# ghostop14/gr-clenabled

Hardware: AMD Instinct MI355X
Metric: MSamples/sec (complex-float) through clFFT 4096 fwd + window + shift (higher is better)
Workload: dtype f32; 1 GPU; BASELINE configs[1]: forward clFFT 4096-pt complex, blackman window + fftshift, 16384 frames/step/GPU device-resident (1 GiB in+out); fft_size=4096, parallelism=replica-per-gpu x1

## Files before the change

### gr-clenabled_amd/csrc/fft_mr.h

```cpp
#pragma once
#include <vector>

#include "common.h"

struct MrPass {
    int radix, ns, nb;
    unsigned m_nb, m_ns;
    int tw_off;
};

struct MrPlan {
    int n = 0, npass = 0;
    int threads = 0;
    int frames = 0;
    int lds_bytes = 0;
    int variant = 0;
    int per_thread = 0;
    MrPass pass[12];
    void *d_tw = nullptr;
};

bool mi355_fft_mr_plan(int n, int sign, int variant, MrPlan *plan, std::vector<float> *tw);

int mi355_fft_mr_tune(MrPlan *plan, mi355_ctx *ctx, int sign, const float *window_dev, float *best_ms);
int mi355_fft_mr_cached_variant(int n);
void mi355_fft_mr_remember(const MrPlan &plan);

int mi355_fft_mr_launch(const MrPlan &plan, mi355_ctx *ctx, int sign, const void *in, void *out, const float *window, int nframes, int shift,
                        int real_in, hipStream_t st);

bool mi355_fft_mr_pfb_ok(const MrPlan &plan, int sign, int K, int M, int nsteps);
int mi355_fft_mr_pfb_launch(const MrPlan &plan, mi355_ctx *ctx, const void *in, void *out, const float *taps, int K, int M, int nsteps, hipStream_t st);
struct MrSynthGeo {
    int threads = 0, frames = 0;
    int nreg = 0, rs = 0;
    int taps_lds = 0, lds_bytes = 0;
};
bool mi355_fft_mr_synth_ok(const MrPlan &plan, int sign, int M, int T, MrSynthGeo *g);
int mi355_fft_mr_synth_launch(const MrPlan &plan, const MrSynthGeo &g, mi355_ctx *ctx, const void *in, void *out, const float *taps_pad,
                              const int *ch_map, int nmap, int T, long long nframes, hipStream_t st);
struct mi355_fft;
const MrPlan *mi355_fft_mr_plan_of(const mi355_fft *h, int *sign);

struct MrTilePlan {
    int n = 0, n1 = 0, n2 = 0;
    MrPlan a, b;
    void *d_twn = nullptr;
};
bool mi355_fft_mr_tile_plan(int n, int sign, MrTilePlan *tp, std::vector<float> *twa, std::vector<float> *twb);
int mi355_fft_mr_tile_launch(const MrTilePlan &tp, mi355_ctx *ctx, int sign, const void *in, void *ws, void *out, const float *window, int nframes,
                             int shift, int real_in, hipStream_t st);
```

### gr-clenabled_amd/csrc/fft_mr.hip

```cpp
#include "fft_mr.h"

#include <cmath>
#include <cstdlib>
#include <map>
#include <mutex>
#include <utility>

#include "fft_core.hpp"
#include "synth_fir.hpp"

using namespace fftc;

namespace {

typedef float f2v __attribute__((ext_vector_type(2)));
constexpr int kVals = 16;
constexpr int kMaxPass = 12;

struct MrArgs {
    const void *in;
    c32 *out;
    const float *window;
    const c32 *tw;
    int n, nframes, frames, npass, in_rot, out_rot, real_in;
    int copy_in = 0;
    int copy_out = 0;
    unsigned m_n = 0;
    int tw_lds = 0, ntw = 0;
    int dbg = 0;
    int fs_shift = 0;
    long long range_len = 0;
    long long ngroups;
    MrPass pass[kMaxPass];
};

__device__ __forceinline__ int slot(int i) { return i + (i >> 5); }

template <int R> __host__ __device__ constexpr int fac_a() { return R == 6 ? 2 : R == 9 ? 3 : R == 10 ? 2 : R == 12 ? 4 : R == 14 ? 2 : R == 15 ? 3 : 1; }
template <int R> __host__ __device__ constexpr int out_index(int s)
{
    if (R == 8 || R == 16) return orev<R>(s);
    if (fac_a<R>() > 1) return s / (R / fac_a<R>()) + fac_a<R>() * (s % (R / fac_a<R>()));
    return s;
}

template <int R> struct Roots;
template <> struct Roots<6> {
    static constexpr float c[6] = {1.000000000e+00f, 5.000000000e-01f, -5.000000000e-01f, -1.000000000e+00f, -5.000000000e-01f, 5.000000000e-01f};
    static constexpr float s[6] = {0.000000000e+00f, 8.660254038e-01f, 8.660254038e-01f, 1.224646799e-16f, -8.660254038e-01f, -8.660254038e-01f};
};
template <> struct Roots<9> {
    static constexpr float c[9] = {1.000000000e+00f, 7.660444431e-01f, 1.736481777e-01f, -5.000000000e-01f, -9.396926208e-01f, -9.396926208e-01f, -5.000000000e-01f, 1.736481777e-01f, 7.660444431e-01f};
    static constexpr float s[9] = {0.000000000e+00f, 6.427876097e-01f, 9.848077530e-01f, 8.660254038e-01f, 3.420201433e-01f, -3.420201433e-01f, -8.660254038e-01f, -9.848077530e-01f, -6.427876097e-01f};
};
template <> struct Roots<10> {
    static constexpr float c[10] = {1.000000000e+00f, 8.090169944e-01f, 3.090169944e-01f, -3.090169944e-01f, -8.090169944e-01f, -1.000000000e+00f, -8.090169944e-01f, -3.090169944e-01f, 3.090169944e-01f, 8.090169944e-01f};
    static constexpr float s[10] = {0.000000000e+00f, 5.877852523e-01f, 9.510565163e-01f, 9.510565163e-01f, 5.877852523e-01f, 1.224646799e-16f, -5.877852523e-01f, -9.510565163e-01f, -9.510565163e-01f, -5.877852523e-01f};
};
template <> struct Roots<12> {
    static constexpr float c[12] = {1.000000000e+00f, 8.660254038e-01f, 5.000000000e-01f, 6.123233996e-17f, -5.000000000e-01f, -8.660254038e-01f, -1.000000000e+00f, -8.660254038e-01f, -5.000000000e-01f, -1.836970199e-16f, 5.000000000e-01f, 8.660254038e-01f};
    static constexpr float s[12] = {0.000000000e+00f, 5.000000000e-01f, 8.660254038e-01f, 1.000000000e+00f, 8.660254038e-01f, 5.000000000e-01f, 1.224646799e-16f, -5.000000000e-01f, -8.660254038e-01f, -1.000000000e+00f, -8.660254038e-01f, -5.000000000e-01f};
};
template <> struct Roots<14> {
    static constexpr float c[14] = {1.000000000e+00f, 9.009688679e-01f, 6.234898019e-01f, 2.225209340e-01f, -2.225209340e-01f, -6.234898019e-01f, -9.009688679e-01f, -1.000000000e+00f, -9.009688679e-01f, -6.234898019e-01f, -2.225209340e-01f, 2.225209340e-01f, 6.234898019e-01f, 9.009688679e-01f};
    static constexpr float s[14] = {0.000000000e+00f, 4.338837391e-01f, 7.818314825e-01f, 9.749279122e-01f, 9.749279122e-01f, 7.818314825e-01f, 4.338837391e-01f, 1.224646799e-16f, -4.338837391e-01f, -7.818314825e-01f, -9.749279122e-01f, -9.749279122e-01f, -7.818314825e-01f, -4.338837391e-01f};
};
template <> struct Roots<15> {
    static constexpr float c[15] = {1.000000000e+00f, 9.135454576e-01f, 6.691306064e-01f, 3.090169944e-01f, -1.045284633e-01f, -5.000000000e-01f, -8.090169944e-01f, -9.781476007e-01f, -9.781476007e-01f, -8.090169944e-01f, -5.000000000e-01f, -1.045284633e-01f, 3.090169944e-01f, 6.691306064e-01f, 9.135454576e-01f};
    static constexpr float s[15] = {0.000000000e+00f, 4.067366431e-01f, 7.431448255e-01f, 9.510565163e-01f, 9.945218954e-01f, 8.660254038e-01f, 5.877852523e-01f, 2.079116908e-01f, -2.079116908e-01f, -5.877852523e-01f, -8.660254038e-01f, -9.945218954e-01f, -9.510565163e-01f, -7.431448255e-01f, -4.067366431e-01f};
};

template <> struct Roots<11> {
    static constexpr float c[11] = {1.000000000e+00f, 8.412535328e-01f, 4.154150130e-01f, -1.423148383e-01f, -6.548607339e-01f, -9.594929736e-01f, -9.594929736e-01f, -6.548607339e-01f, -1.423148383e-01f, 4.154150130e-01f, 8.412535328e-01f};
    static constexpr float s[11] = {0.000000000e+00f, 5.406408175e-01f, 9.096319954e-01f, 9.898214419e-01f, 7.557495744e-01f, 2.817325568e-01f, -2.817325568e-01f, -7.557495744e-01f, -9.898214419e-01f, -9.096319954e-01f, -5.406408175e-01f};
};
template <> struct Roots<13> {
    static constexpr float c[13] = {1.000000000e+00f, 8.854560257e-01f, 5.680647467e-01f, 1.205366803e-01f, -3.546048870e-01f, -7.485107482e-01f, -9.709418174e-01f, -9.709418174e-01f, -7.485107482e-01f, -3.546048870e-01f, 1.205366803e-01f, 5.680647467e-01f, 8.854560257e-01f};
    static constexpr float s[13] = {0.000000000e+00f, 4.647231720e-01f, 8.229838659e-01f, 9.927088741e-01f, 9.350162427e-01f, 6.631226582e-01f, 2.393156643e-01f, -2.393156643e-01f, -6.631226582e-01f, -9.350162427e-01f, -9.927088741e-01f, -8.229838659e-01f, -4.647231720e-01f};
};

template <int R, int SIGN> __device__ __forceinline__ void dft(c32 *v)
{
    if constexpr (R == 2) bfly2<SIGN>(v[0], v[1]);
    else if constexpr (R == 4) bfly4<SIGN>(v[0], v[1], v[2], v[3]);
    else if constexpr (R == 8) bfly8<SIGN>(v);
    else if constexpr (R == 16) bfly16<SIGN>(v);
    else if constexpr (R == 3) {
        constexpr float s3 = 0.86602540378443864676f;
        const c32 t = v[1] + v[2], d = rot90<SIGN>(scale(v[1] - v[2], s3));
        const c32 m = mk(v[0].x - 0.5f * t.x, v[0].y - 0.5f * t.y);
        v[0] = v[0] + t;
        v[1] = m + d;
        v[2] = m - d;
    } else if constexpr (R == 5) {
        constexpr float c1 = 0.30901699437494742410f, c2 = -0.80901699437494742410f, s1 = 0.95105651629515357212f, s2 = 0.58778525229247312917f;
        const c32 t1 = v[1] + v[4], t2 = v[2] + v[3], t3 = v[1] - v[4], t4 = v[2] - v[3];
        const c32 a1 = mk(v[0].x + c1 * t1.x + c2 * t2.x, v[0].y + c1 * t1.y + c2 * t2.y);
        const c32 a2 = mk(v[0].x + c2 * t1.x + c1 * t2.x, v[0].y + c2 * t1.y + c1 * t2.y);
        const c32 b1 = rot90<SIGN>(mk(s1 * t3.x + s2 * t4.x, s1 * t3.y + s2 * t4.y));
        const c32 b2 = rot90<SIGN>(mk(s2 * t3.x - s1 * t4.x, s2 * t3.y - s1 * t4.y));
        v[0] = v[0] + t1 + t2;
        v[1] = a1 + b1;
        v[4] = a1 - b1;
        v[2] = a2 + b2;
        v[3] = a2 - b2;
    } else if constexpr (fac_a<R>() > 1) {
        constexpr int A = fac_a<R>(), B = R / A;
#pragma unroll
        for (int b = 0; b < B; b++) {
            c32 t[A];
#pragma unroll
            for (int q = 0; q < A; q++) t[q] = v[B * q + b];
            dft<A, SIGN>(t);
#pragma unroll
            for (int k1 = 0; k1 < A; k1++) {
                c32 y = t[k1];
                if (b * k1 != 0) {
                    constexpr float sg = SIGN < 0 ? -1.f : 1.f;
                    y = cmul(y, mk(Roots<R>::c[(b * k1) % R], sg * Roots<R>::s[(b * k1) % R]));
                }
                v[B * k1 + b] = y;
            }
        }
#pragma unroll
        for (int k1 = 0; k1 < A; k1++) dft<B, SIGN>(&v[B * k1]);
    } else if constexpr (R == 11 || R == 13) {
        constexpr int H = (R - 1) / 2;
        c32 t[H], u[H];
#pragma unroll
        for (int j = 0; j < H; j++) {
            t[j] = v[j + 1] + v[R - 1 - j];
            u[j] = v[j + 1] - v[R - 1 - j];
        }
        c32 x0 = v[0], sum = v[0];
#pragma unroll
        for (int j = 0; j < H; j++) sum = sum + t[j];
        v[0] = sum;
#pragma unroll
        for (int k = 1; k <= H; k++) {
            c32 ak = x0, bk = mk(0.f, 0.f);
#pragma unroll
            for (int j = 1; j <= H; j++) {
                const float c = Roots<R>::c[(j * k) % R], sn = Roots<R>::s[(j * k) % R];
                ak = mk(ak.x + c * t[j - 1].x, ak.y + c * t[j - 1].y);
                bk = mk(bk.x + sn * u[j - 1].x, bk.y + sn * u[j - 1].y);
            }
            const c32 jb = rot90<SIGN>(bk);
            v[k] = ak + jb;
            v[R - k] = ak - jb;
        }
    } else {
        static_assert(R == 7, "radix");
        constexpr float c1 = 0.62348980185873353053f, c2 = -0.22252093395631440429f, c3 = -0.90096886790241912624f;
        constexpr float s1 = 0.78183148246802980871f, s2 = 0.97492791218182360702f, s3 = 0.43388373911755812048f;
        const c32 t1 = v[1] + v[6], t2 = v[2] + v[5], t3 = v[3] + v[4], u1 = v[1] - v[6], u2 = v[2] - v[5], u3 = v[3] - v[4];
        const c32 a1 = mk(v[0].x + c1 * t1.x + c2 * t2.x + c3 * t3.x, v[0].y + c1 * t1.y + c2 * t2.y + c3 * t3.y);
        const c32 a2 = mk(v[0].x + c2 * t1.x + c3 * t2.x + c1 * t3.x, v[0].y + c2 * t1.y + c3 * t2.y + c1 * t3.y);
        const c32 a3 = mk(v[0].x + c3 * t1.x + c1 * t2.x + c2 * t3.x, v[0].y + c3 * t1.y + c1 * t2.y + c2 * t3.y);
        const c32 b1 = rot90<SIGN>(mk(s1 * u1.x + s2 * u2.x + s3 * u3.x, s1 * u1.y + s2 * u2.y + s3 * u3.y));
        const c32 b2 = rot90<SIGN>(mk(s2 * u1.x - s3 * u2.x - s1 * u3.x, s2 * u1.y - s3 * u2.y - s1 * u3.y));
        const c32 b3 = rot90<SIGN>(mk(s3 * u1.x - s1 * u2.x + s2 * u3.x, s3 * u1.y - s1 * u2.y + s2 * u3.y));
        v[0] = v[0] + t1 + t2 + t3;
        v[1] = a1 + b1;
        v[6] = a1 - b1;
        v[2] = a2 + b2;
        v[5] = a2 - b2;
        v[3] = a3 + b3;
        v[4] = a3 - b3;
    }
}

template <int R, int SIGN, int MODE, bool TWL = false>
__device__ __forceinline__ void mr_pass(const MrArgs &a, const MrPass &ps, c32 *lds, int tid, long long group)
{
    const int TH = blockDim.x;
    constexpr int B = kVals / R;
    c32 v[B][R], w1[B];
    const int n = a.n, nb = ps.nb, nbt = a.frames * nb;
#pragma unroll
    for (int i = 0; i < B; i++) {
        const int b = tid + TH * i;
        const int fr = (int)__umulhi((unsigned)b, ps.m_nb), bb = b - fr * nb;
        if constexpr (MODE == 1 || MODE == 2) {
            const int k = bb - (int)__umulhi((unsigned)bb, ps.m_ns) * ps.ns;
            if constexpr (TWL) w1[i] = b < nbt ? lds[a.tw_lds + ps.tw_off + k] : mk(1.f, 0.f);
            else
            w1[i] = b < nbt ? a.tw[ps.tw_off + k] : mk(1.f, 0.f);
        }
        if (b < nbt) {
            if constexpr (MODE == 0) {
                const long long frame = group * a.frames + fr;
                const bool live = frame < a.nframes;
#pragma unroll
                for (int r = 0; r < R; r++) {
                    int src = bb + r * nb + a.in_rot;
                    if (src >= n) src -= n;
                    c32 x = mk(0.f, 0.f);
                    if (live) {
                        if (a.real_in) x = mk(((const float *)a.in)[(size_t)frame * n + src], 0.f);
                        else {
                            const f2v t = __builtin_nontemporal_load((const f2v *)a.in + (size_t)frame * n + src);
                            x = mk(t.x, t.y);
                        }
                        const float w = a.window[src];
                        x = mk(x.x * w, x.y * w);
                    }
                    v[i][r] = x;
                }
            } else {
                const int base = fr * n + bb;
#pragma unroll
                for (int r = 0; r < R; r++) v[i][r] = lds[slot(base + r * nb)];
            }
        }
    }
    if constexpr (MODE != 0) __syncthreads();
#pragma unroll
    for (int i = 0; i < B; i++) {
        const int b = tid + TH * i;
        if (b < nbt) {
            const int fr = (int)__umulhi((unsigned)b, ps.m_nb), bb = b - fr * nb;
            int g = bb, k = 0;
            if constexpr (MODE == 1 || MODE == 2) {
                g = (int)__umulhi((unsigned)bb, ps.m_ns);
                k = bb - g * ps.ns;
                c32 sq[4];
                sq[0] = w1[i];
#pragma unroll
                for (int q = 1; q < 4; q++) sq[q] = (R > (1 << q)) ? cmul(sq[q - 1], sq[q - 1]) : sq[q - 1];
#pragma unroll
                for (int r = 1; r < R; r++) {
                    c32 t = mk(1.f, 0.f);
                    bool first = true;
#pragma unroll
                    for (int q = 0; q < 4; q++)
                        if ((r >> q) & 1) {
                            t = first ? sq[q] : cmul(t, sq[q]);
                            first = false;
                        }
                    v[i][r] = cmul(v[i][r], t);
                }
            }
            dft<R, SIGN>(v[i]);
            if constexpr (MODE == 2) {
                const long long frame = a.fs_shift ? group + (fr >> a.fs_shift) * a.range_len + (fr & ((1 << a.fs_shift) - 1)) : group * a.frames + fr;
                if (frame < a.nframes) {
#pragma unroll
                    for (int s = 0; s < R; s++) {
                        int p = k + out_index<R>(s) * ps.ns - a.out_rot;
                        if (p < 0) p += n;
                        f2v z;
                        z.x = v[i][s].x;
                        z.y = v[i][s].y;
                        __builtin_nontemporal_store(z, (f2v *)a.out + (size_t)frame * n + p);
                    }
                }
            } else {
                const int base = fr * n + g * ps.ns * R + k;
#pragma unroll
                for (int s = 0; s < R; s++) lds[slot(base + out_index<R>(s) * ps.ns)] = v[i][s];
            }
        }
    }
    if constexpr (MODE != 2) __syncthreads();
}

template <int SIGN>
__global__ __launch_bounds__(1024) void k_fft_mr(const MrArgs a)
{
    extern __shared__ __attribute__((aligned(16))) c32 mr_lds[];
    const int tid0 = threadIdx.x;
#define MR_PASS(MODE, P)                                                                        \
    switch (a.pass[P].radix) {                                                                  \
    case 2: mr_pass<2, SIGN, MODE>(a, a.pass[P], mr_lds, tid, group); break;                \
    case 3: mr_pass<3, SIGN, MODE>(a, a.pass[P], mr_lds, tid, group); break;                \
    case 4: mr_pass<4, SIGN, MODE>(a, a.pass[P], mr_lds, tid, group); break;                \
    case 5: mr_pass<5, SIGN, MODE>(a, a.pass[P], mr_lds, tid, group); break;                \
    case 7: mr_pass<7, SIGN, MODE>(a, a.pass[P], mr_lds, tid, group); break;                \
    case 6: mr_pass<6, SIGN, MODE>(a, a.pass[P], mr_lds, tid, group); break;                    \
    case 9: mr_pass<9, SIGN, MODE>(a, a.pass[P], mr_lds, tid, group); break;                    \
    case 10: mr_pass<10, SIGN, MODE>(a, a.pass[P], mr_lds, tid, group); break;                  \
    case 11: mr_pass<11, SIGN, MODE>(a, a.pass[P], mr_lds, tid, group); break;                  \
    case 13: mr_pass<13, SIGN, MODE>(a, a.pass[P], mr_lds, tid, group); break;                  \
    case 12: mr_pass<12, SIGN, MODE>(a, a.pass[P], mr_lds, tid, group); break;                  \
    case 14: mr_pass<14, SIGN, MODE>(a, a.pass[P], mr_lds, tid, group); break;                  \
    case 15: mr_pass<15, SIGN, MODE>(a, a.pass[P], mr_lds, tid, group); break;                  \
    case 8: mr_pass<8, SIGN, MODE>(a, a.pass[P], mr_lds, tid, group); break;                \
    default: mr_pass<16, SIGN, MODE>(a, a.pass[P], mr_lds, tid, group); break;              \
    }
    for (long long group = blockIdx.x; group < a.ngroups; group += gridDim.x) {
        int tid = tid0;
        asm volatile("" : "+v"(tid));
        if (a.copy_in) {
            const int tot = a.frames * a.n;
            for (int idx = tid0; idx < tot; idx += blockDim.x) {
                const int fr = (int)__umulhi((unsigned)idx, a.m_n), q = idx - fr * a.n;
                int i = q - a.in_rot;
                if (i < 0) i += a.n;
                c32 x = mk(0.f, 0.f);
                if (group * a.frames + fr < a.nframes) {
                    const size_t at = (size_t)group * a.frames * a.n + idx;
                    if (a.real_in) x = mk(((const float *)a.in)[at], 0.f);
                    else {
                        const f2v t = __builtin_nontemporal_load((const f2v *)a.in + at);
                        x = mk(t.x, t.y);
                    }
                    const float w = a.window[q];
                    x = mk(x.x * w, x.y * w);
                }
                mr_lds[slot(fr * a.n + i)] = x;
            }
            __syncthreads();
            MR_PASS(3, 0)
        } else {
            MR_PASS(0, 0)
        }
        for (int p = 1; p < a.npass - 1; p++) { MR_PASS(1, p) }
        if (a.copy_out) {
            MR_PASS(1, a.npass - 1)
            const int tot = a.frames * a.n;
            for (int idx = tid0; idx < tot; idx += blockDim.x) {
                const int fr = (int)__umulhi((unsigned)idx, a.m_n);
                int p = idx - fr * a.n + a.out_rot;
                if (p >= a.n) p -= a.n;
                if (group * a.frames + fr < a.nframes) {
                    const c32 v = mr_lds[slot(fr * a.n + p)];
                    f2v z;
                    z.x = v.x;
                    z.y = v.y;
                    __builtin_nontemporal_store(z, (f2v *)a.out + (size_t)group * a.frames * a.n + idx);
                }
            }
            __syncthreads();
        } else {
            MR_PASS(2, a.npass - 1)
        }
    }
#undef MR_PASS
}


struct PfbMr {
    const c32 *in;
    const float *taps;
    int K, M, Q, nsteps, direct;
    unsigned m_M, m_run;
};

template <int SIGN, int PMAX, int FS>
__global__ __launch_bounds__(512) void k_pfb_mr(const MrArgs a, const PfbMr f)
{
    extern __shared__ __attribute__((aligned(16))) c32 mr_lds[];
    const int tid0 = threadIdx.x;
    const int q = (int)__umulhi((unsigned)tid0, f.m_M), j = tid0 - q * f.M;
    const bool arm = q < f.Q;
// ... 380 lines not shown
}
}

namespace {
bool plan_len(int n, int sign, int variant, bool column_of_a_tile, MrPlan *plan, std::vector<float> *tw);
}

bool mi355_fft_mr_plan(int n, int sign, int variant, MrPlan *plan, std::vector<float> *tw)
{
    if ((n & (n - 1)) == 0) return false;
    return plan_len(n, sign, variant, false, plan, tw);
}

namespace {
bool plan_len(int n, int sign, int variant, bool column_of_a_tile, MrPlan *plan, std::vector<float> *tw)
{
    if (n < 4 || n > 16 * 1024) return false;
    Factorisation fz;
    {
        int cur[kMaxPass];
        search(n, n, 0, 0, kVals, variant ? 14 : 0, cur, &fz);
    }
    if (fz.np > kMaxPass) return false;
    int radix[kMaxPass], np = 0;
    for (int pass = 0; pass < 2; pass++)
        for (int i = 0; i < fz.np; i++) {
            const bool pow2 = (fz.r[i] & (fz.r[i] - 1)) == 0;
            if ((pass == 0) != pow2) radix[np++] = fz.r[i];
        }
    int per_thread = kVals;
    for (int p = 0; p < np; p++) {
        const int v = (kVals / radix[p]) * radix[p];
        if (v < per_thread) per_thread = v;
    }
    int th = 0, frames = 0;
    long long best = 0;
    for (int w : {8, 6, 5, 4, 3, 2, 1}) {
        int t = w == 1 ? 1024 : 1536 / w / 64 * 64;
        long long f = (long long)t * per_thread / n;
        const long long lds_vals = (160 * 1024 / w / 8 - 1) * 32 / 33;
        if (f > lds_vals / n) f = lds_vals / n;
        if (f < 1) continue;
        if (w * f * n > best) {
            best = w * f * n;
            th = t;
            frames = (int)f;
        }
    }
    if (column_of_a_tile) {
        th = (int)((16LL * n + per_thread - 1) / per_thread + 63) / 64 * 64;
        frames = 16;
        if (th > 1024) return false;
    } else
    if (const char *e = getenv("MI355_FFT_MR_THREADS")) {
        const int t = atoi(e), f = getenv("MI355_FFT_MR_FRAMES") ? atoi(getenv("MI355_FFT_MR_FRAMES")) : 1;
        if (t >= 64 && t <= 1024 && t % 64 == 0 && f >= 1 && (long long)f * n <= (long long)t * per_thread) { th = t; frames = f; }
    }
    if (!th) return false;
    plan->n = n;
    plan->npass = np;
    plan->threads = th;
    plan->frames = frames;
    plan->lds_bytes = (plan->frames * n + (plan->frames * n >> 5) + 1) * 8;
    plan->per_thread = per_thread;
    plan->variant = variant;
    tw->clear();
    int ns = 1;
    for (int p = 0; p < np; p++) {
        MrPass &ps = plan->pass[p];
        ps.radix = radix[p];
        ps.ns = ns;
        ps.nb = n / radix[p];
        ps.m_nb = magic(ps.nb);
        ps.m_ns = ns > 1 ? magic(ns) : 0;
        ps.tw_off = (int)(tw->size() / 2);
        if (p > 0)
            for (int k = 0; k < ns; k++) {
                const double a = sign * 2.0 * M_PI * (double)k / ((double)ns * radix[p]);
                tw->push_back((float)cos(a));
                tw->push_back((float)sin(a));
            }
        ns *= radix[p];
    }
    return true;
}
}

namespace {
int lds_bytes_for(int n, int frames) { return (frames * n + (frames * n >> 5) + 1) * 8; }

int launch_with(const MrPlan &plan, int threads, int frames, mi355_ctx *ctx, int sign, const void *in, void *out, const float *window, int nframes,
                int shift, int real_in, hipStream_t st)
{
    MrArgs a;
    a.in = in;
    a.out = (c32 *)out;
    a.window = window;
    a.tw = (const c32 *)plan.d_tw;
    a.n = plan.n;
    a.nframes = nframes;
    a.frames = frames;
    a.npass = plan.npass;
    a.in_rot = (sign > 0 && shift) ? plan.n / 2 : 0;
    a.out_rot = (sign < 0 && shift) ? (plan.n + 1) / 2 : 0;
    a.real_in = real_in;
    a.ngroups = ((long long)nframes + frames - 1) / frames;
    for (int p = 0; p < plan.npass; p++) a.pass[p] = plan.pass[p];
    static const bool no_copy_out = getenv("MI355_FFT_MR_NO_COPY_OUT") != nullptr;
    static const int copy_ns = getenv("MI355_FFT_MR_COPY_OUT_NS") ? atoi(getenv("MI355_FFT_MR_COPY_OUT_NS")) : 32;
    if (no_copy_out) MI355_SWITCH_NOTE(ctx, "MI355_FFT_MR_NO_COPY_OUT", "k_fft_mr with the passes' own loads and stores");
    if (copy_ns != 32) MI355_SWITCH_NOTE(ctx, "MI355_FFT_MR_COPY_OUT_NS", "another run length below which k_fft_mr stores through LDS");
    a.copy_out = plan.pass[plan.npass - 1].ns < copy_ns && !no_copy_out;
    a.m_n = magic(plan.n);
    static const int copy_nb = getenv("MI355_FFT_MR_COPY_IN_NB") ? atoi(getenv("MI355_FFT_MR_COPY_IN_NB")) : 16;
    if (copy_nb != 16) MI355_SWITCH_NOTE(ctx, "MI355_FFT_MR_COPY_IN_NB", "another run length below which k_fft_mr loads through LDS");
    a.copy_in = plan.pass[0].nb < copy_nb && !no_copy_out;
    const int cus = mi355_cus(ctx);
    const int lds_bytes = lds_bytes_for(plan.n, frames);
    int per_cu = (160 * 1024) / lds_bytes;
    if (per_cu > 2048 / threads) per_cu = 2048 / threads;
    if (per_cu < 1) per_cu = 1;
    long long grid = (long long)cus * per_cu;
    if (grid > a.ngroups) grid = a.ngroups;
    static std::map<int, bool> lds_ok;
    static std::mutex lds_ok_lock;
    {
        std::lock_guard<std::mutex> g(lds_ok_lock);
        const int which = ctx->device * 2 + (sign < 0 ? 0 : 1);
        if (!lds_ok[which]) {
            if (sign < 0) MI355_HIP(hipFuncSetAttribute((const void *)k_fft_mr<-1>, hipFuncAttributeMaxDynamicSharedMemorySize, 160 * 1024));
            else MI355_HIP(hipFuncSetAttribute((const void *)k_fft_mr<1>, hipFuncAttributeMaxDynamicSharedMemorySize, 160 * 1024));
            lds_ok[which] = true;
        }
    }
#define MR_LAUNCH(SG) hipLaunchKernelGGL((k_fft_mr<SG>), dim3((unsigned)grid), dim3(threads), lds_bytes, st, a)
    if (sign < 0) MR_LAUNCH(-1); else MR_LAUNCH(1);
#undef MR_LAUNCH
    MI355_HIP(hipGetLastError());
    return MI355_OK;
}

std::mutex g_tuned_lock;
struct Tuned { int variant, threads, frames; };
std::map<int, Tuned> g_tuned;
}

int mi355_fft_mr_launch(const MrPlan &plan, mi355_ctx *ctx, int sign, const void *in, void *out, const float *window, int nframes, int shift,
                        int real_in, hipStream_t st)
{
    if (nframes <= 0) return MI355_OK;
    return launch_with(plan, plan.threads, plan.frames, ctx, sign, in, out, window, nframes, shift, real_in, st);
}

bool mi355_fft_mr_pfb_ok(const MrPlan &plan, int sign, int K, int M, int nsteps)
{
    if (!plan.n || plan.n != M || sign <= 0 || plan.npass < 2 || getenv("MI355_PFB_NO_MR_FUSED")) return false;
    const int P = (K + M - 1) / M;
    return P <= 32 && M <= 512 && (long long)plan.per_thread * 512 >= 8LL * M && nsteps >= 1;
}

int mi355_fft_mr_pfb_launch(const MrPlan &plan, mi355_ctx *ctx, const void *in, void *out, const float *taps, int K, int M, int nsteps, hipStream_t st)
{
    constexpr int FS = 8, FS_SHIFT = 3;
    const int P = (K + M - 1) / M;
    static const int th_env = getenv("MI355_PFB_MR_THREADS") ? atoi(getenv("MI355_PFB_MR_THREADS")) : 0;
    auto ranges_of = [&](int th) { const long long byv = (long long)th * plan.per_thread / (FS * M); const int byt = th / M; return (int)(byv < byt ? byv : byt); };
    if (th_env) MI355_SWITCH_NOTE(ctx, "MI355_PFB_MR_THREADS", "k_pfb_mr with a forced workgroup size");
    int th = 512;
    if (th_env >= 64 && th_env <= 512 && th_env % 64 == 0 && ranges_of(th_env) >= 1) th = th_env;
    const int Q = ranges_of(th);
    if (Q < 1) return MI355_ERR_INVALID_ARG;
    const int cus = mi355_cus(ctx);
    int ntw = 0;
    for (int p = 1; p < plan.npass; p++) ntw += plan.pass[p].ns;
    const int tw_lds = lds_bytes_for(M, Q * FS) / 8;
    const int pmax = P <= 8 ? 8 : P <= 16 ? 16 : 32;
    const int lds_bytes = (tw_lds + ntw) * 8 + pmax * M * 4;
    static const int wg_env = getenv("MI355_PFB_MR_WG_PER_CU") ? atoi(getenv("MI355_PFB_MR_WG_PER_CU")) : 0;
    if (wg_env > 0) MI355_SWITCH_NOTE(ctx, "MI355_PFB_MR_WG_PER_CU", "k_pfb_mr with a forced number of workgroups per CU");
    int per_cu = wg_env > 0 ? wg_env : (pmax == 8 ? 16 : 12) / (th / 64);
    if (per_cu > (160 * 1024) / lds_bytes) per_cu = (160 * 1024) / lds_bytes;
    if (per_cu < 1) per_cu = 1;
    long long len = (nsteps + (long long)cus * Q - 1) / ((long long)cus * Q);
    if (len >= 8LL * P) {
        const long long nr = (long long)cus * per_cu * Q;
        len = (nsteps + nr - 1) / nr;
        if (len < 8LL * P) len = 8LL * P;
    }
    len = (len + FS - 1) / FS * FS;
    const long long grid = (nsteps + len * Q - 1) / (len * Q);
    MrArgs a;
    a.in = nullptr;
    a.out = (c32 *)out;
    a.window = nullptr;
    a.tw = (const c32 *)plan.d_tw;
    a.n = M;
    a.nframes = nsteps;
    a.frames = Q * FS;
    a.npass = plan.npass;
    a.in_rot = a.out_rot = a.real_in = 0;
    a.fs_shift = FS_SHIFT;
    a.range_len = len;
    a.tw_lds = tw_lds;
    a.ntw = ntw;
    a.dbg = getenv("MI355_PFB_MR_DBG") ? atoi(getenv("MI355_PFB_MR_DBG")) : 0;
    a.ngroups = 0;
    for (int p = 0; p < plan.npass; p++) a.pass[p] = plan.pass[p];
    PfbMr f;
    f.in = (const c32 *)in;
    f.taps = taps;
    f.K = K;
    f.M = M;
    f.Q = Q;
    f.nsteps = nsteps;
    f.m_M = magic(M);
    f.m_run = magic(FS * M);
    f.direct = (a.dbg & 32) ? 1 : (a.dbg & 16) ? 0 : plan.pass[plan.npass - 1].ns >= 8;
    if (lds_bytes > 160 * 1024) return MI355_ERR_INVALID_ARG;
    if (lds_bytes > 48 * 1024) {
        static std::map<int, bool> lds_ok;
        static std::mutex lds_ok_lock;
        std::lock_guard<std::mutex> g(lds_ok_lock);
        if (!lds_ok[ctx->device]) {
            MI355_HIP(hipFuncSetAttribute((const void *)k_pfb_mr<1, 8, FS>, hipFuncAttributeMaxDynamicSharedMemorySize, 160 * 1024));
            MI355_HIP(hipFuncSetAttribute((const void *)k_pfb_mr<1, 16, FS>, hipFuncAttributeMaxDynamicSharedMemorySize, 160 * 1024));
            MI355_HIP(hipFuncSetAttribute((const void *)k_pfb_mr<1, 32, FS>, hipFuncAttributeMaxDynamicSharedMemorySize, 160 * 1024));
            lds_ok[ctx->device] = true;
        }
    }
#define PFB_MR(PM) hipLaunchKernelGGL((k_pfb_mr<1, PM, FS>), dim3((unsigned)grid), dim3(th), lds_bytes, st, a, f)
    if (pmax == 8) PFB_MR(8); else if (pmax == 16) PFB_MR(16); else PFB_MR(32);
#undef PFB_MR
    MI355_HIP(hipGetLastError());
    return MI355_OK;
// ... 11 lines not shown
    for (int F = (int)fmax; F >= 1; F--) {
        const long long nreg = 1 + ((long long)T - 1 + F - 1) / F, rs = lds_bytes_for(M, F) / 8, ring = nreg * rs * 8;
        if (ring > 160 * 1024) continue;
        g->threads = th;
        g->frames = F;
        g->nreg = (int)nreg;
        g->rs = (int)rs;
        g->taps_lds = ring + (long long)T * M * 4 <= 160 * 1024;
        g->lds_bytes = (int)(ring + (g->taps_lds ? (long long)T * M * 4 : 0));
        return true;
    }
    return false;
}

int mi355_fft_mr_synth_launch(const MrPlan &plan, const MrSynthGeo &g, mi355_ctx *ctx, const void *in, void *out, const float *taps_pad,
                              const int *ch_map, int nmap, int T, long long nframes, hipStream_t st)
{
    if (nframes <= 0) return MI355_OK;
    const int M = plan.n, F = g.frames;
    const int cus = mi355_cus(ctx);
    int per_cu = (160 * 1024) / g.lds_bytes;
    if (per_cu > 2048 / g.threads) per_cu = 2048 / g.threads;
    if (per_cu < 1) per_cu = 1;
    const long long ntiles = (nframes + F - 1) / F, cap = (long long)cus * per_cu;
    const long long minrun = g.nreg > 1 ? 4LL * (g.nreg - 1) : 1;
    long long grid = (ntiles + minrun - 1) / minrun;
    if (grid > cap) grid = cap;
    const long long per = (ntiles + grid - 1) / grid;
    grid = (ntiles + per - 1) / per;
    MrArgs a;
    a.in = nullptr;
    a.out = nullptr;
    a.window = nullptr;
    a.tw = (const c32 *)plan.d_tw;
    a.n = M;
    a.nframes = 0;
    a.frames = F;
    a.npass = plan.npass;
    a.in_rot = a.out_rot = a.real_in = 0;
    a.ngroups = 0;
    for (int p = 0; p < plan.npass; p++) a.pass[p] = plan.pass[p];
    SynMr f;
    f.in = (const c32 *)in;
    f.out = (f2v *)out;
    f.taps = taps_pad;
    f.ch_map = ch_map;
    f.nmap = nmap;
    f.T = T;
    f.nreg = g.nreg;
    f.rs = g.rs;
    f.taps_lds = g.taps_lds;
    f.per = (int)per;
    f.nframes = nframes;
    f.nin_items = ((long long)T - 1 + nframes) * nmap;
    f.ntiles = ntiles;
    f.m_M = magic(M);
    if (g.lds_bytes > 48 * 1024) {
        static std::map<int, bool> lds_ok;
        static std::mutex lds_ok_lock;
        std::lock_guard<std::mutex> lk(lds_ok_lock);
        if (!lds_ok[ctx->device]) {
            MI355_HIP(hipFuncSetAttribute((const void *)k_synth_mr<1>, hipFuncAttributeMaxDynamicSharedMemorySize, 160 * 1024));
            lds_ok[ctx->device] = true;
        }
    }
    hipLaunchKernelGGL((k_synth_mr<1>), dim3((unsigned)grid), dim3(g.threads), (size_t)g.lds_bytes, st, a, f);
    MI355_HIP(hipGetLastError());
    return MI355_OK;
}

int mi355_fft_mr_tune(MrPlan *plan, mi355_ctx *ctx, int sign, const float *window_dev, float *best_ms_out)
{
    const int per_thread = plan->per_thread;
    if (best_ms_out) *best_ms_out = -1.f;
    if (const char *e = getenv("MI355_FFT_MR_AUTOTUNE"))
        if (atoi(e) == 0) return MI355_OK;
    if (getenv("MI355_FFT_MR_THREADS")) return MI355_OK;
    {
        std::lock_guard<std::mutex> g(g_tuned_lock);
        auto it = g_tuned.find(plan->n);
        if (it != g_tuned.end() && it->second.variant == plan->variant) {
            plan->threads = it->second.threads;
            plan->frames = it->second.frames;
            plan->lds_bytes = lds_bytes_for(plan->n, plan->frames);
            return MI355_OK;
        }
    }
    const int n = plan->n;
    const size_t total = (size_t)1 << 23;
    const int nframes = (int)(total / n);
    void *din = nullptr, *dout = nullptr;
    if (hipMalloc(&din, (size_t)nframes * n * 8) != hipSuccess) { (void)hipGetLastError(); return MI355_OK; }
    if (hipMalloc(&dout, (size_t)nframes * n * 8) != hipSuccess) { (void)hipGetLastError(); (void)hipFree(din); return MI355_OK; }
    std::lock_guard<std::mutex> g(ctx->upload_lock);
    hipStream_t st = ctx->upload;
    hipEvent_t e0 = nullptr, e1 = nullptr;
    int rc = MI355_OK;
    auto done = [&](int r) {
        if (e0) (void)hipEventDestroy(e0);
        if (e1) (void)hipEventDestroy(e1);
        (void)hipFree(din);
        (void)hipFree(dout);
        if (r == MI355_OK) (void)hipGetLastError();
        return r;
    };
    if (hipEventCreate(&e0) != hipSuccess || hipEventCreate(&e1) != hipSuccess) return done(MI355_OK);
    if (hipMemsetAsync(din, 0, (size_t)nframes * n * 8, st) != hipSuccess) return done(MI355_OK);
    float best_ms = 1e30f;
    int best_t = plan->threads, best_f = plan->frames;
    auto trial = [&](int t, int f) {
        if (f < 1 || (long long)f * n > (long long)t * per_thread || lds_bytes_for(n, f) > 160 * 1024) return;
        if (launch_with(*plan, t, f, ctx, sign, din, dout, window_dev, nframes, 0, 0, st) != MI355_OK) { rc = MI355_ERR_HIP; return; }
        float ms = 1e30f;
        for (int rep = 0; rep < 2; rep++) {
            (void)hipEventRecord(e0, st);
            for (int k = 0; k < 3; k++)
                if (launch_with(*plan, t, f, ctx, sign, din, dout, window_dev, nframes, 0, 0, st) != MI355_OK) { rc = MI355_ERR_HIP; return; }
            (void)hipEventRecord(e1, st);
            if (hipEventSynchronize(e1) != hipSuccess) { rc = MI355_ERR_HIP; return; }
            float m = 0.f;
            if (hipEventElapsedTime(&m, e0, e1) != hipSuccess) return;
            if (m < ms) ms = m;
        }
        if (ms < best_ms * 0.98f) {
            best_ms = ms;
            best_t = t;
            best_f = f;
        }
    };
    trial(plan->threads, plan->frames);
    for (int t = 64; t <= 1024 && rc == MI355_OK; t += 64) {
        const int fmax = (int)((long long)t * per_thread / n);
        if (fmax < 1) continue;
        int tried[4] = {fmax, (fmax * 3 + 3) / 4, (fmax + 1) / 2, 1}, ntried = 0;
        for (int f : tried) {
            bool dup = false;
            for (int q = 0; q < ntried; q++) dup = dup || tried[q] == f;
            if (!dup && rc == MI355_OK) trial(t, f);
            tried[ntried++] = f;
        }
    }
    if (rc != MI355_OK) return done(rc);
    plan->threads = best_t;
    plan->frames = best_f;
    plan->lds_bytes = lds_bytes_for(n, best_f);
    if (best_ms_out) *best_ms_out = best_ms;
    return done(MI355_OK);
}

int mi355_fft_mr_cached_variant(int n)
{
    std::lock_guard<std::mutex> g(g_tuned_lock);
    auto it = g_tuned.find(n);
    return it == g_tuned.end() ? -1 : it->second.variant;
}

void mi355_fft_mr_remember(const MrPlan &plan)
{
    std::lock_guard<std::mutex> g(g_tuned_lock);
    g_tuned[plan.n] = Tuned{plan.variant, plan.threads, plan.frames};
}

namespace {
int tile_fs(int n) { return n | 1; }
int tile_lds_bytes(int n) { const int v = 16 * tile_fs(n); return (v + (v >> 5) + 1) * 8; }
}

bool mi355_fft_mr_tile_plan(int n, int sign, MrTilePlan *tp, std::vector<float> *twa, std::vector<float> *twb)
{
    if (n <= 15360 || n > 960 * 960) return false;
    double best = 1e30;
    MrPlan pa, pb;
    std::vector<float> ta, tb;
    for (int n1 = 4; n1 <= 960; n1++) {
        if (n % n1) continue;
        const int n2 = n / n1;
        if (n2 < 4 || n2 > 960) continue;
        bool ok = false;
        for (int va = 0; va < 2 && !ok; va++)
            for (int vb = 0; vb < 2 && !ok; vb++)
                ok = plan_len(n1, sign, va, true, &pa, &ta) && plan_len(n2, sign, vb, true, &pb, &tb) && tile_lds_bytes(n1) <= 160 * 1024 &&
                     tile_lds_bytes(n2) <= 160 * 1024;
        if (!ok) continue;
        double cost = pa.npass + pb.npass + (n2 % 16 ? 0.5 : 0.0) + (n1 % 16 ? 0.5 : 0.0) + 0.25 * fabs(log2((double)n1 / n2));
        if (cost < best) {
            best = cost;
            tp->n = n;
            tp->n1 = n1;
            tp->n2 = n2;
            tp->a = pa;
            tp->b = pb;
            *twa = ta;
            *twb = tb;
        }
    }
    return best < 1e29;
}

int mi355_fft_mr_tile_launch(const MrTilePlan &tp, mi355_ctx *ctx, int sign, const void *in, void *ws, void *out, const float *window, int nframes,
                             int shift, int real_in, hipStream_t st)
{
    if (nframes <= 0) return MI355_OK;
    static std::map<int, bool> lds_ok;
    static std::mutex lds_ok_lock;
    {
        std::lock_guard<std::mutex> g(lds_ok_lock);
        const int which = ctx->device * 2 + (sign < 0 ? 0 : 1);
        if (!lds_ok[which]) {
            if (sign < 0) {
                MI355_HIP(hipFuncSetAttribute((const void *)k_fft_mr_tile<-1, false>, hipFuncAttributeMaxDynamicSharedMemorySize, 160 * 1024));
                MI355_HIP(hipFuncSetAttribute((const void *)k_fft_mr_tile<-1, true>, hipFuncAttributeMaxDynamicSharedMemorySize, 160 * 1024));
            } else {
                MI355_HIP(hipFuncSetAttribute((const void *)k_fft_mr_tile<1, false>, hipFuncAttributeMaxDynamicSharedMemorySize, 160 * 1024));
                MI355_HIP(hipFuncSetAttribute((const void *)k_fft_mr_tile<1, true>, hipFuncAttributeMaxDynamicSharedMemorySize, 160 * 1024));
            }
            lds_ok[which] = true;
        }
    }
    const int cus = mi355_cus(ctx);
    for (int pass = 0; pass < 2; pass++) {
        const MrPlan &pl = pass ? tp.b : tp.a;
        TileArgs a;
        a.in = pass ? ws : in;
        a.out = (c32 *)(pass ? out : ws);
        a.window = pass ? nullptr : window;
        a.tw = (const c32 *)pl.d_tw;
        a.twn = (const c32 *)tp.d_twn;
        a.n = pl.n;
        a.ld = pass ? tp.n1 : tp.n2;
        a.big = tp.n;
        a.nframes = nframes;
        a.npass = pl.npass;
        a.in_rot = (!pass && sign > 0 && shift) ? tp.n / 2 : 0;
        a.out_rot = (pass && sign < 0 && shift) ? (tp.n + 1) / 2 : 0;
        a.real_in = pass ? 0 : real_in;
        a.fs = tile_fs(pl.n);
        a.nt = a.ld % 16 == 0 && a.in_rot % 16 == 0 && a.out_rot % 16 == 0;
        a.nitems = (long long)nframes * ((a.ld + 15) / 16);
        for (int p = 0; p < pl.npass; p++) a.pass[p] = pl.pass[p];
        const int lds_bytes = tile_lds_bytes(pl.n);
        int per_cu = (160 * 1024) / lds_bytes;
        if (per_cu > 2048 / pl.threads) per_cu = 2048 / pl.threads;
        if (per_cu < 1) per_cu = 1;
// ... 14 lines not shown
```

Baseline: 390,800 MSamples/s.

## Prefetch next frame group via buffer loads in persistent multi-radix FFT kernel

Adds a prefetching variant of the multi-radix FFT kernel. The persistent loop issues buffer loads for the next group's input before running the current group's LDS passes, keeps the window in registers, stages twiddles in LDS, and writes output with bounds-checked buffer stores. The aim is to hide global memory latency behind compute. A residency rule and the autotuner choose between the prefetch and plain kernels, trading extra register pressure and LDS for the overlap.

```diff
diff --git a/gr-clenabled_amd/csrc/fft_mr.h b/gr-clenabled_amd/csrc/fft_mr.h
--- a/gr-clenabled_amd/csrc/fft_mr.h
+++ b/gr-clenabled_amd/csrc/fft_mr.h
@@ -16,11 +16,15 @@
     int lds_bytes = 0;
     int variant = 0;
     int per_thread = 0;
+    int ntw = 0;
+    int prefetch = 0;
     MrPass pass[12];
     void *d_tw = nullptr;
 };
 
 bool mi355_fft_mr_plan(int n, int sign, int variant, MrPlan *plan, std::vector<float> *tw);
+
+bool mi355_fft_mr_prefetch_rule(int n, int threads, int frames, int per_thread, int ntw);
 
 int mi355_fft_mr_tune(MrPlan *plan, mi355_ctx *ctx, int sign, const float *window_dev, float *best_ms);
 int mi355_fft_mr_cached_variant(int n);
diff --git a/gr-clenabled_amd/csrc/fft_mr.hip b/gr-clenabled_amd/csrc/fft_mr.hip
--- a/gr-clenabled_amd/csrc/fft_mr.hip
+++ b/gr-clenabled_amd/csrc/fft_mr.hip
@@ -27,6 +27,8 @@
     int copy_out = 0;
     unsigned m_n = 0;
     int tw_lds = 0, ntw = 0;
+    unsigned m_r0 = 0;
+    int vals0 = 0;
     int dbg = 0;
     int fs_shift = 0;
     long long range_len = 0;
@@ -170,13 +172,31 @@
     }
 }
 
-template <int R, int SIGN, int MODE, bool TWL = false>
-__device__ __forceinline__ void mr_pass(const MrArgs &a, const MrPass &ps, c32 *lds, int tid, long long group)
-{
+typedef unsigned u2v __attribute__((ext_vector_type(2)));
+
+__device__ __forceinline__ __amdgpu_buffer_rsrc_t group_rsrc(const void *base, long long group, const MrArgs &a, int esz)
+{
+    long long live = (long long)a.nframes - group * a.frames;
+    live = live < 0 ? 0 : live > a.frames ? a.frames : live;
+    const char *p = (const char *)base + (live ? (size_t)group * a.frames * a.n * esz : 0);
+    return __builtin_amdgcn_make_buffer_rsrc((void *)p, 0, (int)(live * a.n * esz), 0x00020000);
+}
+
+template <int R, int SIGN, int MODE, bool TWL = false, bool BUF = false>
+__device__ __forceinline__ void mr_pass(const MrArgs &a, const MrPass &ps, c32 *lds, int tid, long long group, c32 *sv = nullptr, unsigned *so = nullptr)
+{
+    static_assert(!BUF || MODE == 2, "buffer stores: the last pass");
     const int TH = blockDim.x;
     constexpr int B = kVals / R;
     c32 v[B][R], w1[B];
     const int n = a.n, nb = ps.nb, nbt = a.frames * nb;
+    if constexpr (BUF) {
+#pragma unroll
+        for (int q = B * R; q < kVals; q++) {
+            sv[q] = mk(0.f, 0.f);
+            so[q] = 0x80000000u;
+        }
+    }
 #pragma unroll
     for (int i = 0; i < B; i++) {
         const int b = tid + TH * i;
@@ -212,13 +232,16 @@
 #pragma unroll
                 for (int r = 0; r < R; r++) v[i][r] = lds[slot(base + r * nb)];
             }
+        } else if constexpr (BUF) {
+#pragma unroll
+            for (int r = 0; r < R; r++) v[i][r] = mk(0.f, 0.f);
         }
     }
     if constexpr (MODE != 0) __syncthreads();
 #pragma unroll
     for (int i = 0; i < B; i++) {
         const int b = tid + TH * i;
-        if (b < nbt) {
+        if (BUF || b < nbt) {
             const int fr = (int)__umulhi((unsigned)b, ps.m_nb), bb = b - fr * nb;
             int g = bb, k = 0;
             if constexpr (MODE == 1 || MODE == 2) {
@@ -242,7 +265,15 @@
                 }
             }
             dft<R, SIGN>(v[i]);
-            if constexpr (MODE == 2) {
+            if constexpr (BUF) {
+#pragma unroll
+                for (int s = 0; s < R; s++) {
+                    int p = k + out_index<R>(s) * ps.ns - a.out_rot;
+                    if (p < 0) p += n;
+                    sv[i * R + s] = v[i][s];
+                    so[i * R + s] = (unsigned)(fr * n + p) * 8u;
+                }
+            } else if constexpr (MODE == 2) {
                 const long long frame = a.fs_shift ? group + (fr >> a.fs_shift) * a.range_len + (fr & ((1 << a.fs_shift) - 1)) : group * a.frames + fr;
                 if (frame < a.nframes) {
 #pragma unroll
@@ -265,12 +296,192 @@
     if constexpr (MODE != 2) __syncthreads();
 }
 
+__device__ __forceinline__ int mr_where(const MrArgs &a, int tid, int v)
+{
+    constexpr int none = 1 << 28;
+    const int TH = blockDim.x;
+    if (a.copy_in) {
+        const int idx = tid + TH * v;
+        return idx < a.frames * a.n ? idx : none;
+    }
+    const MrPass &ps = a.pass[0];
+    const int i = (int)__umulhi((unsigned)v, a.m_r0), r = v - i * ps.radix;
+    const int b = tid + TH * i;
+    const int fr = (int)__umulhi((unsigned)b, ps.m_nb), bb = b - fr * ps.nb;
+    int src = bb + r * ps.nb + a.in_rot;
+    if (src >= a.n) src -= a.n;
+    return v < a.vals0 && b < a.frames * ps.nb ? fr * a.n + src : none;
+}
+
+__device__ __forceinline__ void mr_issue(const MrArgs &a, int tid, long long group, f2v *pf)
+{
+    const __amdgpu_buffer_rsrc_t rs = group_rsrc(a.in, group, a, a.real_in ? 4 : 8);
+    if (a.real_in) {
+#pragma unroll
+        for (int v = 0; v < kVals; v++) pf[v].x = __builtin_bit_cast(float, __builtin_amdgcn_raw_buffer_load_b32(rs, (unsigned)mr_where(a, tid, v) * 4u, 0, 0));
+    } else {
+#pragma unroll
+        for (int v = 0; v < kVals; v++)
+            pf[v] = __builtin_bit_cast(f2v, __builtin_amdgcn_raw_buffer_load_b64(rs, (unsigned)mr_where(a, tid, v) * 8u, 0, 2 ));
+    }
+}
+
+__device__ __forceinline__ void mr_window(const MrArgs &a, int tid, float *wreg)
+{
+#pragma unroll
+    for (int v = 0; v < kVals; v++) {
+        const int at = mr_where(a, tid, v);
+        float w = 0.f;
+        if (at < (1 << 28)) w = a.window[at - (int)__umulhi((unsigned)at, a.m_n) * a.n];
+        wreg[v] = w;
+    }
+}
+
+__device__ __forceinline__ c32 mr_windowed(const MrArgs &a, f2v x, float w)
+{
+    float re = x.x * w, im = (a.real_in ? 0.f : x.y) * w;
+    asm("" : "+v"(re), "+v"(im));
+    return mk(re, im);
+}
+
+template <int R, int SIGN>
+__device__ __forceinline__ void mr_first(const MrArgs &a, const MrPass &ps, c32 *lds, int tid, const f2v *pf, const float *wreg)
+{
+    const int TH = blockDim.x;
+    constexpr int B = kVals / R;
+    const int n = a.n, nb = ps.nb, nbt = a.frames * nb;
+#pragma unroll
+    for (int i = 0; i < B; i++) {
+        const int b = tid + TH * i;
+        if (b < nbt) {
+            const int fr = (int)__umulhi((unsigned)b, ps.m_nb), bb = b - fr * nb;
+            c32 v[R];
+#pragma unroll
+            for (int r = 0; r < R; r++) v[r] = mr_windowed(a, pf[i * R + r], wreg[i * R + r]);
+            dft<R, SIGN>(v);
+            const int base = fr * n + bb * ps.ns * R;
+#pragma unroll
+            for (int s = 0; s < R; s++) lds[slot(base + out_index<R>(s) * ps.ns)] = v[s];
+        }
+    }
+    __syncthreads();
+}
+
 template <int SIGN>
+__device__ __forceinline__ void mr_groups_prefetched(const MrArgs &a, c32 *mr_lds)
+{
+    const int tid0 = threadIdx.x;
+    f2v pf[kVals];
+    float wreg[kVals];
+    mr_window(a, tid0, wreg);
+    for (int i = tid0; i < a.ntw; i += blockDim.x) mr_lds[a.tw_lds + i] = a.tw[i];
+    __syncthreads();
+#pragma unroll
+    for (int v = 0; v < kVals; v++) asm volatile("" : "+v"(wreg[v]));
+#pragma unroll
+    for (int v = 0; v < kVals; v++) pf[v] = f2v{0.f, 0.f};
+    mr_issue(a, tid0, blockIdx.x, pf);
+#pragma unroll
+    for (int v = 0; v < kVals; v++) asm volatile("" : "+v"(pf[v]));
+#define MR_PASS(MODE, P, BUF)                                                                   \
+    switch (a.pass[P].radix) {                                                                  \
+    case 2: mr_pass<2, SIGN, MODE, true, BUF>(a, a.pass[P], mr_lds, tid, group, sv, so); break; \
+    case 3: mr_pass<3, SIGN, MODE, true, BUF>(a, a.pass[P], mr_lds, tid, group, sv, so); break;         \
+    case 4: mr_pass<4, SIGN, MODE, true, BUF>(a, a.pass[P], mr_lds, tid, group, sv, so); break;         \
+    case 5: mr_pass<5, SIGN, MODE, true, BUF>(a, a.pass[P], mr_lds, tid, group, sv, so); break;         \
+    case 7: mr_pass<7, SIGN, MODE, true, BUF>(a, a.pass[P], mr_lds, tid, group, sv, so); break;         \
+    case 6: mr_pass<6, SIGN, MODE, true, BUF>(a, a.pass[P], mr_lds, tid, group, sv, so); break;         \
+    case 9: mr_pass<9, SIGN, MODE, true, BUF>(a, a.pass[P], mr_lds, tid, group, sv, so); break;         \
+    case 10: mr_pass<10, SIGN, MODE, true, BUF>(a, a.pass[P], mr_lds, tid, group, sv, so); break;       \
+    case 11: mr_pass<11, SIGN, MODE, true, BUF>(a, a.pass[P], mr_lds, tid, group, sv, so); break;       \
+    case 13: mr_pass<13, SIGN, MODE, true, BUF>(a, a.pass[P], mr_lds, tid, group, sv, so); break;       \
+    case 12: mr_pass<12, SIGN, MODE, true, BUF>(a, a.pass[P], mr_lds, tid, group, sv, so); break;       \
+    case 14: mr_pass<14, SIGN, MODE, true, BUF>(a, a.pass[P], mr_lds, tid, group, sv, so); break;       \
+    case 15: mr_pass<15, SIGN, MODE, true, BUF>(a, a.pass[P], mr_lds, tid, group, sv, so); break;       \
+    case 8: mr_pass<8, SIGN, MODE, true, BUF>(a, a.pass[P], mr_lds, tid, group, sv, so); break;         \
+    default: mr_pass<16, SIGN, MODE, true, BUF>(a, a.pass[P], mr_lds, tid, group, sv, so); break;       \
+    }
+#define MR_FIRST                                                                                \
+    switch (a.pass[0].radix) {                                                                  \
+    case 2: mr_first<2, SIGN>(a, a.pass[0], mr_lds, tid, pf, wreg); break;                      \
+    case 3: mr_first<3, SIGN>(a, a.pass[0], mr_lds, tid, pf, wreg); break;                      \
+    case 4: mr_first<4, SIGN>(a, a.pass[0], mr_lds, tid, pf, wreg); break;                      \
+    case 5: mr_first<5, SIGN>(a, a.pass[0], mr_lds, tid, pf, wreg); break;                      \
+    case 7: mr_first<7, SIGN>(a, a.pass[0], mr_lds, tid, pf, wreg); break;                      \
+    case 6: mr_first<6, SIGN>(a, a.pass[0], mr_lds, tid, pf, wreg); break;                      \
+    case 9: mr_first<9, SIGN>(a, a.pass[0], mr_lds, tid, pf, wreg); break;                      \
+    case 10: mr_first<10, SIGN>(a, a.pass[0], mr_lds, tid, pf, wreg); break;                    \
+    case 11: mr_first<11, SIGN>(a, a.pass[0], mr_lds, tid, pf, wreg); break;                    \
+    case 13: mr_first<13, SIGN>(a, a.pass[0], mr_lds, tid, pf, wreg); break;                    \
+    case 12: mr_first<12, SIGN>(a, a.pass[0], mr_lds, tid, pf, wreg); break;                    \
+    case 14: mr_first<14, SIGN>(a, a.pass[0], mr_lds, tid, pf, wreg); break;                    \
+    case 15: mr_first<15, SIGN>(a, a.pass[0], mr_lds, tid, pf, wreg); break;                    \
+    case 8: mr_first<8, SIGN>(a, a.pass[0], mr_lds, tid, pf, wreg); break;                      \
+    default: mr_first<16, SIGN>(a, a.pass[0], mr_lds, tid, pf, wreg); break;                    \
+    }
+    const int tot = a.frames * a.n;
+    for (long long group = blockIdx.x; group < a.ngroups; group += gridDim.x) {
+        int tid = tid0;
+        asm volatile("" : "+v"(tid));
+        c32 sv[kVals];
+        unsigned so[kVals];
+        if (a.copy_in) {
+#pragma unroll
+            for (int u = 0; u < kVals; u++) {
+                const int idx = tid + blockDim.x * u;
+                if (idx < tot) {
+                    const int fr = (int)__umulhi((unsigned)idx, a.m_n);
+                    int i = idx - fr * a.n - a.in_rot;
+                    if (i < 0) i += a.n;
+                    mr_lds[slot(fr * a.n + i)] = mr_windowed(a, pf[u], wreg[u]);
+                }
+            }
+            __syncthreads();
+        } else {
+            MR_FIRST
+        }
+        mr_issue(a, tid, group + gridDim.x, pf);
+        __builtin_amdgcn_sched_barrier(0);
+        if (a.copy_in) { MR_PASS(3, 0, false) }
+        for (int p = 1; p < a.npass - 1; p++) { MR_PASS(1, p, false) }
+        if (a.copy_out) {
+            MR_PASS(1, a.npass - 1, false)
+#pragma unroll
+            for (int u = 0; u < kVals; u++) {
+                const int idx = tid + blockDim.x * u;
+                const int fr = (int)__umulhi((unsigned)idx, a.m_n);
+                int p = idx - fr * a.n + a.out_rot;
+                if (p >= a.n) p -= a.n;
+                sv[u] = idx < tot ? mr_lds[slot(fr * a.n + p)] : mk(0.f, 0.f);
+                so[u] = idx < tot ? (unsigned)idx * 8u : 0x80000000u;
+            }
+            __syncthreads();
+        } else {
+            MR_PASS(2, a.npass - 1, true)
+        }
+        const __amdgpu_buffer_rsrc_t ors = group_rsrc((const void *)a.out, group, a, 8);
+#pragma unroll
+        for (int q = 0; q < kVals; q++) {
+            f2v z;
+            z.x = sv[q].x;
+            z.y = sv[q].y;
+            __builtin_amdgcn_raw_buffer_store_b64(__builtin_bit_cast(u2v, z), ors, so[q], 0, 2 );
+        }
+    }
+#undef MR_FIRST
+#undef MR_PASS
+}
+
+template <int SIGN, bool PF = false>
 __global__ __launch_bounds__(1024) void k_fft_mr(const MrArgs a)
 {
     extern __shared__ __attribute__((aligned(16))) c32 mr_lds[];
+    if constexpr (PF) {
+        mr_groups_prefetched<SIGN>(a, mr_lds);
+        return;
+    }
     const int tid0 = threadIdx.x;
-#define MR_PASS(MODE, P)                                                                        \
+#define MR_PASS(MODE, P)                                                                     \
     switch (a.pass[P].radix) {                                                                  \
     case 2: mr_pass<2, SIGN, MODE>(a, a.pass[P], mr_lds, tid, group); break;                \
     case 3: mr_pass<3, SIGN, MODE>(a, a.pass[P], mr_lds, tid, group); break;                \
@@ -817,14 +1028,38 @@
             }
         ns *= radix[p];
     }
+    plan->ntw = (int)(tw->size() / 2);
+    plan->prefetch = !column_of_a_tile && mi355_fft_mr_prefetch_rule(n, th, frames, per_thread, plan->ntw);
+    if (plan->prefetch) plan->lds_bytes += plan->ntw * 8;
     return true;
 }
 }
 
 namespace {
 int lds_bytes_for(int n, int frames) { return (frames * n + (frames * n >> 5) + 1) * 8; }
-
-int launch_with(const MrPlan &plan, int threads, int frames, mi355_ctx *ctx, int sign, const void *in, void *out, const float *window, int nframes,
+int lds_bytes_for(int n, int frames, int ntw, int prefetch) { return lds_bytes_for(n, frames) + (prefetch ? ntw * 8 : 0); }
+constexpr int kMrThreadsPerCu[2] = {1792, 1024};
+int resident_per_cu(int threads, int lds_bytes, int prefetch)
+{
+    const int by_lds = lds_bytes > 0 ? (160 * 1024) / lds_bytes : 0, by_regs = kMrThreadsPerCu[prefetch] / threads;
+    return by_lds < by_regs ? by_lds : by_regs;
+}
+}
+
+#ifndef MI355_FFT_MR_PREFETCH
+#define MI355_FFT_MR_PREFETCH 1
+#endif
+
+bool mi355_fft_mr_prefetch_rule(int n, int threads, int frames, int per_thread, int ntw)
+{
+    if (!MI355_FFT_MR_PREFETCH || threads < 64 || frames < 1 || (long long)frames * n > (long long)threads * per_thread) return false;
+    const int with = resident_per_cu(threads, lds_bytes_for(n, frames, ntw, 1), 1), without = resident_per_cu(threads, lds_bytes_for(n, frames, ntw, 0), 0);
+    return with >= 1 && with >= without;
+}
+
+namespace {
+
+int launch_with(const MrPlan &plan, int threads, int frames, int prefetch, mi355_ctx *ctx, int sign, const void *in, void *out, const float *window, int nframes,
                 int shift, int real_in, hipStream_t st)
 {
     MrArgs a;
@@ -851,9 +1086,15 @@
     if (copy_nb != 16) MI355_SWITCH_NOTE(ctx, "MI355_FFT_MR_COPY_IN_NB", "another run length below which k_fft_mr loads through LDS");
     a.copy_in = plan.pass[0].nb < copy_nb && !no_copy_out;
     const int cus = mi355_cus(ctx);
-    const int lds_bytes = lds_bytes_for(plan.n, frames);
-    int per_cu = (160 * 1024) / lds_bytes;
-    if (per_cu > 2048 / threads) per_cu = 2048 / threads;
+    const int lds_bytes = lds_bytes_for(plan.n, frames, plan.ntw, prefetch);
+    if (prefetch) {
+        if (lds_bytes > 160 * 1024) return MI355_ERR_INVALID_ARG;
+        a.tw_lds = lds_bytes_for(plan.n, frames) / 8;
+        a.ntw = plan.ntw;
+        a.m_r0 = magic(plan.pass[0].radix);
+        a.vals0 = kVals / plan.pass[0].radix * plan.pass[0].radix;
+    }
+    int per_cu = resident_per_cu(threads, lds_bytes, prefetch);
     if (per_cu < 1) per_cu = 1;
     long long grid = (long long)cus * per_cu;
     if (grid > a.ngroups) grid = a.ngroups;
@@ -863,20 +1104,29 @@
         std::lock_guard<std::mutex> g(lds_ok_lock);
         const int which = ctx->device * 2 + (sign < 0 ? 0 : 1);
         if (!lds_ok[which]) {
-            if (sign < 0) MI355_HIP(hipFuncSetAttribute((const void *)k_fft_mr<-1>, hipFuncAttributeMaxDynamicSharedMemorySize, 160 * 1024));
-            else MI355_HIP(hipFuncSetAttribute((const void *)k_fft_mr<1>, hipFuncAttributeMaxDynamicSharedMemorySize, 160 * 1024));
+            if (sign < 0) {
+                MI355_HIP(hipFuncSetAttribute((const void *)k_fft_mr<-1, false>, hipFuncAttributeMaxDynamicSharedMemorySize, 160 * 1024));
+                MI355_HIP(hipFuncSetAttribute((const void *)k_fft_mr<-1, true>, hipFuncAttributeMaxDynamicSharedMemorySize, 160 * 1024));
+            } else {
+                MI355_HIP(hipFuncSetAttribute((const void *)k_fft_mr<1, false>, hipFuncAttributeMaxDynamicSharedMemorySize, 160 * 1024));
+                MI355_HIP(hipFuncSetAttribute((const void *)k_fft_mr<1, true>, hipFuncAttributeMaxDynamicSharedMemorySize, 160 * 1024));
+            }
             lds_ok[which] = true;
         }
     }
-#define MR_LAUNCH(SG) hipLaunchKernelGGL((k_fft_mr<SG>), dim3((unsigned)grid), dim3(threads), lds_bytes, st, a)
-    if (sign < 0) MR_LAUNCH(-1); else MR_LAUNCH(1);
-#undef MR_LAUNCH
+    if (sign < 0) {
+        if (prefetch) hipLaunchKernelGGL((k_fft_mr<-1, true>), dim3((unsigned)grid), dim3(threads), lds_bytes, st, a);
+        else hipLaunchKernelGGL((k_fft_mr<-1, false>), dim3((unsigned)grid), dim3(threads), lds_bytes, st, a);
+    } else {
+        if (prefetch) hipLaunchKernelGGL((k_fft_mr<1, true>), dim3((unsigned)grid), dim3(threads), lds_bytes, st, a);
+        else hipLaunchKernelGGL((k_fft_mr<1, false>), dim3((unsigned)grid), dim3(threads), lds_bytes, st, a);
+    }
     MI355_HIP(hipGetLastError());
     return MI355_OK;
 }
 
 std::mutex g_tuned_lock;
-struct Tuned { int variant, threads, frames; };
+struct Tuned { int variant, threads, frames, prefetch; };
 std::map<int, Tuned> g_tuned;
 }
 
@@ -884,7 +1134,7 @@
                         int real_in, hipStream_t st)
 {
     if (nframes <= 0) return MI355_OK;
-    return launch_with(plan, plan.threads, plan.frames, ctx, sign, in, out, window, nframes, shift, real_in, st);
+    return launch_with(plan, plan.threads, plan.frames, plan.prefetch, ctx, sign, in, out, window, nframes, shift, real_in, st);
 }
 
 bool mi355_fft_mr_pfb_ok(const MrPlan &plan, int sign, int K, int M, int nsteps)
@@ -1062,7 +1312,8 @@
         if (it != g_tuned.end() && it->second.variant == plan->variant) {
             plan->threads = it->second.threads;
             plan->frames = it->second.frames;
-            plan->lds_bytes = lds_bytes_for(plan->n, plan->frames);
+            plan->prefetch = it->second.prefetch;
+            plan->lds_bytes = lds_bytes_for(plan->n, plan->frames, plan->ntw, plan->prefetch);
             return MI355_OK;
         }
     }
@@ -1087,15 +1338,16 @@
     if (hipEventCreate(&e0) != hipSuccess || hipEventCreate(&e1) != hipSuccess) return done(MI355_OK);
     if (hipMemsetAsync(din, 0, (size_t)nframes * n * 8, st) != hipSuccess) return done(MI355_OK);
     float best_ms = 1e30f;
-    int best_t = plan->threads, best_f = plan->frames;
-    auto trial = [&](int t, int f) {
-        if (f < 1 || (long long)f * n > (long long)t * per_thread || lds_bytes_for(n, f) > 160 * 1024) return;
-        if (launch_with(*plan, t, f, ctx, sign, din, dout, window_dev, nframes, 0, 0, st) != MI355_OK) { rc = MI355_ERR_HIP; return; }
+    int best_t = plan->threads, best_f = plan->frames, best_pf = plan->prefetch;
+    auto trial = [&](int t, int f, int pf) {
+        if (f < 1 || (long long)f * n > (long long)t * per_thread || lds_bytes_for(n, f, plan->ntw, pf) > 160 * 1024) return;
+        if (pf && !MI355_FFT_MR_PREFETCH) return;
+        if (launch_with(*plan, t, f, pf, ctx, sign, din, dout, window_dev, nframes, 0, 0, st) != MI355_OK) { rc = MI355_ERR_HIP; return; }
         float ms = 1e30f;
         for (int rep = 0; rep < 2; rep++) {
             (void)hipEventRecord(e0, st);
             for (int k = 0; k < 3; k++)
-                if (launch_with(*plan, t, f, ctx, sign, din, dout, window_dev, nframes, 0, 0, st) != MI355_OK) { rc = MI355_ERR_HIP; return; }
+                if (launch_with(*plan, t, f, pf, ctx, sign, din, dout, window_dev, nframes, 0, 0, st) != MI355_OK) { rc = MI355_ERR_HIP; return; }
             (void)hipEventRecord(e1, st);
             if (hipEventSynchronize(e1) != hipSuccess) { rc = MI355_ERR_HIP; return; }
             float m = 0.f;
@@ -1106,9 +1358,10 @@
             best_ms = ms;
             best_t = t;
             best_f = f;
+            best_pf = pf;
         }
     };
-    trial(plan->threads, plan->frames);
+    trial(plan->threads, plan->frames, plan->prefetch);
     for (int t = 64; t <= 1024 && rc == MI355_OK; t += 64) {
         const int fmax = (int)((long long)t * per_thread / n);
         if (fmax < 1) continue;
@@ -1116,14 +1369,16 @@
         for (int f : tried) {
             bool dup = false;
             for (int q = 0; q < ntried; q++) dup = dup || tried[q] == f;
-            if (!dup && rc == MI355_OK) trial(t, f);
+            for (int pf = 0; pf < 2; pf++)
+                if (!dup && rc == MI355_OK) trial(t, f, pf);
             tried[ntried++] = f;
         }
     }
     if (rc != MI355_OK) return done(rc);
     plan->threads = best_t;
     plan->frames = best_f;
-    plan->lds_bytes = lds_bytes_for(n, best_f);
+    plan->prefetch = best_pf;
+    plan->lds_bytes = lds_bytes_for(n, best_f, plan->ntw, best_pf);
     if (best_ms_out) *best_ms_out = best_ms;
     return done(MI355_OK);
 }
@@ -1138,7 +1393,7 @@
 void mi355_fft_mr_remember(const MrPlan &plan)
 {
     std::lock_guard<std::mutex> g(g_tuned_lock);
-    g_tuned[plan.n] = Tuned{plan.variant, plan.threads, plan.frames};
+    g_tuned[plan.n] = Tuned{plan.variant, plan.threads, plan.frames, plan.prefetch};
 }
 
 namespace {
```

New measurement: 390,700 MSamples/s. Within noise of the previous version (-0.0%).
